# liruiw/OMG-Planner

Measured on AMD Instinct MI355X. Metric: CHOMP iterations/sec (batched scenes) + ms/plan, Panda 7-DoF 30-wp, higher is better.
Workload: dtype f32 SDF / f64 kinematics+update; 1 GPU; 100 table-top scenes/GPU x (64-goal goal-set cost + CHOMP step), Panda 9-dof, 30 waypoints; scenes_per_gpu=100, total_scenes=100, goals=64, waypoints=30, sdf_grid=4x64^3 + 128x96x32 per scene, private, goal_selection=MD on device (omgx_goal_update_optimize), pipeline_parts=3, top_k_collision=1000, plan_restart_every_steps=50

## Files before the change

### include/omg_hip.h

```cpp
#ifndef OMG_HIP_H
#define OMG_HIP_H

#include <stdint.h>

#ifdef __cplusplus
extern "C" {
#endif

#define OMGX_OK 0
#define OMGX_ERR_INVALID (-1)
#define OMGX_ERR_LAUNCH (-2)
#define OMGX_ERR_UNSUPPORTED (-3)

#define OMGX_NUM_LINKS 10
#define OMGX_NUM_DOF 9
#define OMGX_MAX_POINTS 16
#define OMGX_MAX_WAYPOINTS 64
#define OMGX_MAX_CONSTRAINTS 8
#define OMGX_INFO_STRIDE 16

#define OMGX_ROBOT_POSE0 0
#define OMGX_ROBOT_TIP2JOINT 160
#define OMGX_ROBOT_CENTER_OFFSET 320
#define OMGX_ROBOT_JOINT_AXIS 480
// ... 188 lines not shown
                         const int32_t* h_dims, float* out, void* stream);

int32_t omgx_goalset_schedule_len(int32_t num_scenes, int32_t num_goals, int32_t slack);
int omgx_goalset_schedule(const uint32_t* work, const int32_t* active, const int32_t* goal_count, int32_t num_scenes,
                          int32_t num_goals, int32_t slack, int32_t* schedule, void* stream);

int omgx_goalset_schedule_parts(const uint32_t* work, const int32_t* active, const int32_t* goal_count, int32_t num_scenes,
                                int32_t num_goals, int32_t parts, int32_t slack, int32_t* schedule, void* stream);

#define OMGX_SCHEDULE_SCENE_MAJOR 0
#define OMGX_SCHEDULE_LONGEST_FIRST 1
#define OMGX_SCHEDULE_LONGEST_FIRST_MAX_ITEMS 8192
int omgx_goalset_schedule_ordered(const uint32_t* work, const int32_t* active, const int32_t* goal_count, int32_t num_scenes,
                                  int32_t num_goals, int32_t parts, int32_t slack, int32_t order, int32_t* schedule, void* stream);

int64_t omgx_region_scratch_bytes(int32_t dx, int32_t dy, int32_t dz);
int omgx_object_set_grid(omgx_object* object, const float* h_lo, const float* h_hi, const int32_t* h_dims, float delta,
                         int64_t grid_offset, void* stream);
int omgx_fit_influence_region(omgx_object* object, const float* grid, const int32_t* h_dims, const float* h_lo, const float* h_hi,
                              float epsilon, float clearance, void* scratch, void* stream);

int64_t omgx_regions_scratch_bytes(int32_t n_fit, int64_t need_bytes);
int omgx_volume_hashes(const omgx_object* objects, int32_t num_objects, const float* pool, uint64_t* hashes, void* stream);
int omgx_fit_influence_regions(omgx_object* objects, int32_t num_objects, const float* pool, const int32_t* fit_list,
                               const int64_t* need_offsets, int32_t n_fit, int64_t max_voxels, const int32_t* copy_src,
                               void* scratch, void* stream);

typedef struct omgx_plan_iter {
    int32_t mode;
    int32_t start_idx;
// ... 105 lines not shown
```

### omg-planner_amd/csrc/omg_goalset_queue.h

```cpp
#pragma once

#define GQ_TBL_MAX 32
#ifndef GQ_WG_PER_CU
#define GQ_WG_PER_CU 5
#endif
#ifndef GQ_WAVES
#define GQ_WAVES 4
#endif
#define GQ_NT (64 * GQ_WAVES)

struct GqFar {
    float T[12], lo[3], rc[3], rh[3], rr2, rb_r;
    bool cullable;
    int disabled;
};

typedef uint32_t GqU16 __attribute__((ext_vector_type(16)));
typedef uint32_t GqU8 __attribute__((ext_vector_type(8)));
typedef uint32_t GqU4 __attribute__((ext_vector_type(4)));
static_assert(offsetof(omgx_object, pose_inv) == 0 && offsetof(omgx_object, lo) == 0x30 && offsetof(omgx_object, epsilon) == 0x58 &&
              offsetof(omgx_object, clearance) == 0x60 && offsetof(omgx_object, disabled) == 0x64 && offsetof(omgx_object, rb_c) == 0x88 &&
              offsetof(omgx_object, rb_h) == 0x94 && offsetof(omgx_object, rb_r) == 0xa0 && offsetof(omgx_object, rb_r2) == 0xa4 &&
              sizeof(omgx_object) >= 0xa8, "gq_load_far reads the record by byte offsets");
__device__ __forceinline__ GqFar gq_load_far(ObjTablePtr ob) {
// ... 75 lines not shown
    e[12] = __float_as_uint(r.eps); e[13] = __float_as_uint(r.clr);
    e[14] = __float_as_uint(r.pad); e[15] = __float_as_uint(r.i2e);
}

template <bool PERSIST>
__device__ __forceinline__ double gq_ld_traj(const double* p) {
    if constexpr (PERSIST) return __hip_atomic_load(p, __ATOMIC_RELAXED, __HIP_MEMORY_SCOPE_AGENT);
    else return *p;
}
template <bool PERSIST>
__device__ __forceinline__ void gq_st_out(float* p, float v) {
    if constexpr (PERSIST) __hip_atomic_store(p, v, __ATOMIC_RELAXED, __HIP_MEMORY_SCOPE_AGENT);
    else *p = v;
}

template <int LB, bool STAMP, bool LAT, bool SPLIT, bool PRE, bool PERSIST = false, int ROLE = 0, int W = GQ_WAVES, bool RANGE = false>
__device__ __forceinline__ void gq_item(const ChunkArgs& a, double* const lds_pose, const int s, const bool is_layer, const int layer_part, const int chunk, const int NP) {
    const int o_begin = as_const(a.scene_begin)[s], o_end = as_const(a.scene_begin)[s + 1];
    const int P = a.P;
    const bool warming = LAT && o_end > o_begin;
    const int goal = NP > 1 ? chunk / NP : chunk;
    const int part = NP > 1 ? chunk - goal * NP : 0;
    static_assert(!RANGE || (SPLIT && !LAT && !PRE && !PERSIST && W == GQ_WAVES), "waypoint ranges: the batch kernel with two parts per goal and their own kinematics");
    const int CHg = a.CH;
    const int cfg_off = (RANGE && part > 0) ? a.range_h : 0;
    const int CH = RANGE ? (part > 0 ? CHg - a.range_h : a.range_h) : CHg;
    const int blk_shift = (4 - (CH & 3)) & 3;
    const int p = threadIdx.x & 15, lane = threadIdx.x & 63;
    const int wave = __builtin_amdgcn_readfirstlane((int)(threadIdx.x >> 6));
    const int tid = (int)threadIdx.x;
    const RobotViewS rv(a.robot, P);
    const int pstride = a.PS, MR = a.MR;
    static_assert(W == GQ_WAVES || (!LAT && !SPLIT && !PRE && !PERSIST && W >= 4), "wide workgroups: the batch kernel with whole goals and its own kinematics");
    constexpr int NT = 64 * W;
    const GqLayout L(pstride, MR, P, a.tbl_n, LAT, W);
    char* const lds_bytes = reinterpret_cast<char*>(lds_pose);
    uint32_t* const rowmask = reinterpret_cast<uint32_t*>(lds_bytes + L.mask_off);
    uint32_t* const tilebits = reinterpret_cast<uint32_t*>(lds_bytes + L.tile_off);
    if (ROLE == 1 || (ROLE == 0 && is_layer)) {
        const int lgi = a.layer_nb > 1 ? layer_part / a.layer_nb : layer_part, cbi = layer_part - lgi * a.layer_nb;
        const int lpg = 10 / a.layer_lg, c_begin = cbi * a.layer_cb;
        const int c_end = c_begin + a.layer_cb < a.wp_n ? c_begin + a.layer_cb : a.wp_n;
        waypoint_layer_block<LAT, PERSIST>(a, s, lgi * lpg, (lgi + 1) * lpg, c_begin, c_end, lds_pose, rowmask, o_begin, o_end, rv,
                                  reinterpret_cast<double*>(lds_bytes + L.fkc_off), warming,
                                  reinterpret_cast<float*>(lds_bytes + L.objc_off), reinterpret_cast<double*>(lds_bytes + L.btab_off));
        GS_WG_STAMP(4);
        return;
    }
    if (a.goal_count && goal >= as_const(a.goal_count)[s]) {
        if (STAMP && tid == 0) a.work[(int64_t)s * a.NCH + chunk] = 0u;
        return;
    }
    const unsigned long long work_t0 = STAMP ? wall_clock64() : 0ull;
    GS_FREQ_BEGIN();
    uint32_t* const tbl = reinterpret_cast<uint32_t*>(lds_bytes + L.tbl_off);
    double* const pts = reinterpret_cast<double*>(lds_bytes + L.pts_off);
    float* const stage = reinterpret_cast<float*>(lds_bytes + L.stage_off) + wave * 256;

    auto cull_row = [&](int l, int ci) {
        const double* A = lds_pose + 9 + ((int64_t)l * pstride + ci) * 9;
        const auto bl = rv.ball(l);
        float cx, cy, cz;
        link_ball_center(A, A + 3, A + 6, bl, cx, cy, cz);
        const float rad = (float)bl[3] + 1.0e-4f;
// ... 58 lines not shown
            for (int j = 0; j < 12; ++j) {
                const int l = lk / 9, k = lk - 9 * l;
                if (e0 + GQ_NT * j < ne) lds_pose[((size_t)l * pstride + c) * 9 + k] = v[j];
                c += dr; lk += dq;
                if (c >= ncfg) { c -= ncfg; ++lk; }
            }
        }
#pragma unroll
        for (int j = 0; j < 3; ++j) if (tid + GQ_NT * j < nm) rowmask[tid + GQ_NT * j] = mv[j];
        if (tid < 30 * P) pts[tid] = pv0;
        if (tid + GQ_NT < 30 * P) pts[tid + GQ_NT] = pv1;
        if (tbl_lane) gq_tbl_store(tbl + (tid - 128) * 16, trec);
        GS_WG_STAMP(1);
    } else
    {
        const double* q0 = a.traj_start + a.ts_stride * (int64_t)s;
        const double* qg = a.goals + ((int64_t)s * a.NG + goal) * 9;
        const int ncfg = CH + 1;
        double* sc = reinterpret_cast<double*>(lds_bytes + L.stage_off);
        int* const progress = reinterpret_cast<int*>(lds_bytes + L.stage_off + pstride * 14 * 8);
        if (tid < 4) progress[tid] = (tid < chain_waves || (cull_beside_chain && tid == 3)) ? 0 : 99;
        const double pv0 = tid < 30 * P ? rv.g[246 + tid] : 0.0, pv1 = (tid < 256 && tid + 256 < 30 * P) ? rv.g[246 + tid + 256] : 0.0;
        double* const fkc = reinterpret_cast<double*>(lds_bytes + L.fkc_off);
        const double fkv = (LAT && tid < 246) ? rv.g[tid] : 0.0;
        const bool tbl_lane = tid >= 128 && tid - 128 < a.tbl_n && o_begin + tid - 128 < o_end;
        GqTblRec trec{};
        if (LAT && tbl_lane) trec = gq_tbl_load(a.objects + o_begin + (tid - 128));
        if (warming) gq_warm_scalar_cache(a.objects, o_begin, o_end, a.robot + OMGX_ROBOT_POINTS + 30 * P + 316 + 30 * P);
        auto joint = [&](int cfg_local, int d) {
            const int cfg = cfg_local + cfg_off;
            const double q0d = gq_ld_traj<PERSIST>(q0 + d);
            return cfg == 0 ? q0d : q0d + ((double)cfg * (1.0 / (double)(CHg + 1))) * (qg[d] - q0d);
        };
        for (int t = tid; t < ncfg * 7; t += NT) {
            const int cfg = t / 7, i = t - cfg * 7;
            double sn, cs;
#ifdef OMGX_GS_PRO2
            {
                double qq = joint(cfg, i);
                asm volatile("" : "+v"(qq));
                fk_joint_sincos(qq, sn, cs);
                asm volatile("" : : "v"(sn), "v"(cs));
            }
#endif
            fk_joint_sincos(joint(cfg, i), sn, cs);
            sc[2 * t] = sn; sc[2 * t + 1] = cs;
        }
        if (LAT && tid < 246) fkc[tid] = fkv;
        __syncthreads();
        GS_WG_STAMP(1);
        if (tid < 30 * P) pts[tid] = pv0;
        if (tid < 256 && tid + 256 < 30 * P) pts[tid + 256] = pv1;
        if (tbl_lane) {
            if (!LAT) trec = gq_tbl_load(a.objects + o_begin + (tid - 128));
            gq_tbl_store(tbl + (tid - 128) * 16, trec);
        }
        auto run_chain = [&](const auto& view) {
            for (int t = tid; t < ncfg * 3; t += NT) {
                const int cfg = t / 3, rr = t - cfg * 3;
                fk_chain_row(view, rr, sc + 14 * cfg, joint(cfg, 7), joint(cfg, 8), [&](int l, double r0, double r1, double r2, double tr) {
// ... 413 lines not shown
template <int W> struct GqWide { static constexpr int wg_per_cu = W == GQ_WAVES ? GQ_WG_PER_CU : (W <= 6 ? 3 : 2); };
template <int LB, bool STAMP, bool LAT, bool SPLIT, bool PRE, int W, bool RANGE>
__device__ __forceinline__ void goalset_queue_body(const ChunkArgs& a, double* const lds_pose) {
    GS_WG_STAMP(0);
#ifdef OMGX_GS_PRIO
    __builtin_amdgcn_s_setprio(OMGX_GS_PRIO);
#endif
    const int xcd = blockIdx.x & 7;
    const int LPARTS = a.layer_parts;
    const bool spread = LAT;
    static_assert(!(LAT && SPLIT), "latency mode has its parts already");
    const int NP = (LAT || SPLIT) ? a.NP : 1;
    bool is_layer;
    int s, chunk, layer_part;
    bool scheduled = false;
    if (spread) {
        const int nl = a.wp_traj ? a.S * LPARTS : 0;
        is_layer = (int)blockIdx.x < nl;
        const int j = (int)blockIdx.x - nl;
        s = is_layer ? (int)blockIdx.x / LPARTS : j / a.NCH;
        layer_part = (int)blockIdx.x - s * LPARTS;
        chunk = is_layer ? 0 : j - s * a.NCH;
    } else {
        const int nlayer = a.wp_traj ? ((a.S + 7) >> 3) * LPARTS : 0;
        is_layer = (int)(blockIdx.x >> 3) < nlayer;
        const int j = (int)(blockIdx.x >> 3) - nlayer;
        const int sgrp = is_layer ? (int)(blockIdx.x >> 3) / LPARTS : j / a.NCH;
        layer_part = (int)(blockIdx.x >> 3) - sgrp * LPARTS;
        s = sgrp * 8 + xcd;
        chunk = is_layer ? 0 : j - sgrp * a.NCH;
        scheduled = a.schedule && !is_layer;
        if (scheduled) {
            const int item = as_const(a.schedule)[(int)blockIdx.x - nlayer * 8];
            if (item < 0 || item >= a.S * a.NCH) return;
            s = item / a.NCH;
            chunk = item - s * a.NCH;
            if (a.active && as_const(a.active)[s] == 0) { if (STAMP && threadIdx.x == 0) a.work[item] = 0u; return; }
        }
    }
    if (s >= a.S) return;
    if (a.active && !scheduled && !spread) {
        const int k = s, ln = threadIdx.x & 63;
        int seen = 0;
        s = -1;
        for (int base = 0; base < a.S; base += 64) {
            const int i = base + ln;
            const unsigned long long bal = __ballot(i < a.S && a.active[i] != 0);
            const int cnt = __popcll(bal);
            if (k < seen + cnt) {
                unsigned long long m = bal;
                for (int q = k - seen; q > 0; --q) m &= m - 1;
                s = base + __builtin_ctzll(m);
                break;
            }
            seen += cnt;
        }
    }
    if (s < 0) return;
    if (spread && a.active && as_const(a.active)[s] == 0) return;
    if constexpr (W != GQ_WAVES) {
        if (is_layer && threadIdx.x >= 64 * GQ_WAVES) return;
    }
    gq_item<LB, STAMP, LAT, SPLIT, PRE, false, 0, W, RANGE>(a, lds_pose, s, is_layer, layer_part, chunk, NP);
}

template <int LB, bool STAMP = false, bool LAT = false, bool SPLIT = false, bool PRE = false, int W = GQ_WAVES>
__global__ __launch_bounds__(LAT ? 256 : 64 * W, LAT ? 2 : GqWide<W>::wg_per_cu) void k_goalset_queue(ChunkArgs a) {
    extern __shared__ __attribute__((aligned(16))) double lds_pose[];
    goalset_queue_body<LB, STAMP, LAT, SPLIT, PRE, W, false>(a, lds_pose);
}

template <int LB, bool STAMP = false>
__global__ __launch_bounds__(GQ_NT, GQ_WG_PER_CU) void k_goalset_range(ChunkArgs a) {
    extern __shared__ __attribute__((aligned(16))) double lds_pose[];
    goalset_queue_body<LB, STAMP, false, true, false, GQ_WAVES, true>(a, lds_pose);
}
```

### omg-planner_amd/csrc/omg_kernels.hip

```cpp
#include <hip/hip_runtime.h>
#include <hip/hip_ext.h>

#include <stdint.h>
#include <stdio.h>
#include <stdlib.h>
#include <string.h>

#include <mutex>

#include "omg_device.h"
#include "omg_host.h"

using namespace omg;

struct RawObjects {
    const float* __restrict__ pose_init;
    const float* __restrict__ sdf_grids;
    const float* __restrict__ sdf_limits;
    const float* __restrict__ eps;
    const float* __restrict__ pad;
    const float* __restrict__ clr;
    const float* __restrict__ dis;
};

// ... 129 lines not shown
    int wp_n, wp_soften;
    float* wp_pot;
    float* wp_grad;
    float* wp_col;
    int PS, MR;
    const int32_t* schedule;
    int sched_len;
    int tbl_n;
    int NG, NP;
    int range_h;
    int layer_parts, layer_lg, layer_nb, layer_cb, spread;
    double* wp_pose_out;
    uint32_t* work;
    double* pre_poses;
    uint32_t* pre_masks;
};

template <bool WANT_GRAD, int LB, bool FUSED, int TPB = 256>
__global__ __launch_bounds__(TPB) void k_sdf_chunks(ChunkArgs a) {
    extern __shared__ __attribute__((aligned(16))) double lds_pose[];
    __shared__ float red[2][TPB / 64];
    uint32_t* rowmask = reinterpret_cast<uint32_t*>(lds_pose + (FUSED ? (size_t)(a.CH + 1) * 120 : 0));
    const int xcd = blockIdx.x & 7;
    const int nlg = 10 / a.LPW;
    const int jj = blockIdx.x >> 3;
    const int j = jj / nlg, lg = jj - j * nlg;
    const int sgrp = j / a.NCH;
    const int s = sgrp * 8 + xcd, chunk = j - sgrp * a.NCH;
    if (s >= a.S) return;
    const int l_begin = lg * a.LPW, l_end = l_begin + a.LPW;
// ... 643 lines not shown
    }
    ca.pre_poses = nullptr; ca.pre_masks = nullptr;
    if (pre) {
        const int64_t goals = (int64_t)ca.S * ca.NG;
        ca.pre_poses = reinterpret_cast<double*>(tl.kin_ws);
        ca.pre_masks = reinterpret_cast<uint32_t*>(ca.pre_poses + goals * gk_pose_doubles(ca.CH));
        const int ncfg = ca.CH + 1, gpw = ncfg <= 64 ? 64 / ncfg : 1;
        const int64_t waves = (int64_t)ca.S * ((ca.NG + gpw - 1) / gpw);
        hipLaunchKernelGGL(k_goalset_kin, dim3((unsigned)((waves + 3) / 4)), dim3(256), 0, st, ca);
        OMGX_CHECK_LAUNCH("k_goalset_kin");
    }
    hipEvent_t ev0, ev1;
    timing_events(timing_kind, &ev0, &ev1);
    const unsigned g = (unsigned)grid;
    uint32_t l32 = (uint32_t)lds;
#ifdef OMGX_GS_CLOCK
    if (const char* e = getenv("OMGX_GS_LDS_MIN")) { const uint32_t v = (uint32_t)atoi(e); if (v > l32 && v <= 64 * 1024) l32 = v; }
#endif
    const auto go = [&](auto* kernel, int block) { gs_launch(kernel, g, (unsigned)block, l32, st, ev0, ev1, ca); };
    if (range) { if (ca.work) go(k_goalset_range<2, true>, GQ_NT); else go(k_goalset_range<2, false>, GQ_NT); }
    else if (wide == 6) { if (ca.work) go(k_goalset_queue<2, true, false, false, false, 6>, 64 * 6); else go(k_goalset_queue<2, false, false, false, false, 6>, 64 * 6); }
    else if (wide == 8) { if (ca.work) go(k_goalset_queue<2, true, false, false, false, 8>, 64 * 8); else go(k_goalset_queue<2, false, false, false, false, 8>, 64 * 8); }
    else if (ca.spread) { if (pre) go(k_goalset_queue<2, false, true, false, true>, 256); else go(k_goalset_queue<2, false, true, false, false>, 256); }
    else if (split && ca.work) { if (pre) go(k_goalset_queue<2, true, false, true, true>, GQ_NT); else go(k_goalset_queue<2, true, false, true, false>, GQ_NT); }
    else if (split) { if (pre) go(k_goalset_queue<2, false, false, true, true>, GQ_NT); else go(k_goalset_queue<2, false, false, true, false>, GQ_NT); }
    else if (ca.work) { if (pre) go(k_goalset_queue<2, true, false, false, true>, GQ_NT); else go(k_goalset_queue<2, true, false, false, false>, GQ_NT); }
    else { if (pre) go(k_goalset_queue<2, false, false, false, true>, GQ_NT); else go(k_goalset_queue<2, false, false, false, false>, GQ_NT); }
    g_last_goalset_variant = (range ? 0x100 : 0) | (split ? 0x200 : 0) | (ca.spread ? 0x400 : 0) | (pre ? 0x800 : 0) | (range ? GQ_WAVES : wide);
    OMGX_CHECK_LAUNCH("k_goalset_queue");
    return OMGX_OK;
// ... 143 lines not shown

struct GoalsetCall {
    const double* robot = nullptr; int32_t n_points = 0;
    const omgx_object* objects = nullptr; const int32_t* scene_begin = nullptr; const float* sdf_pool = nullptr;
    const double* traj_start = nullptr; int64_t traj_start_stride = 0; const double* goals = nullptr;
    int32_t num_scenes = 0, num_goals = 0, n_remaining = 0, soften_fingers = 0;
    double time_interval = 0.0;
    float *goal_cost = nullptr, *collides = nullptr;
    float* potentials = nullptr;
    void* workspace = nullptr;
    const double* layer_traj = nullptr;
    int32_t layer_n = 0, layer_soften = 0;
    float *layer_pot = nullptr, *layer_grad = nullptr, *layer_col = nullptr;
    const int32_t *active = nullptr, *goal_count = nullptr, *schedule = nullptr;
    int32_t schedule_len = 0; uint32_t* work = nullptr;
    void* stream = nullptr;
    GsTiling tiling;
};

static int goalset_cost_impl(const GoalsetCall& a) {
    if (a.num_scenes < 0 || a.num_goals < 0) return OMGX_ERR_INVALID;
    if (a.num_scenes == 0 || (a.num_goals == 0 && !a.layer_traj)) return OMGX_OK;
    if (!a.robot || !a.objects || !a.scene_begin) return OMGX_ERR_INVALID;
    if (a.num_goals > 0 && (!a.traj_start || !a.goals || !a.goal_cost)) return OMGX_ERR_INVALID;
    if (a.n_points < 1 || a.n_points > OMGX_MAX_POINTS || a.n_remaining < 1 || a.n_remaining > OMGX_MAX_WAYPOINTS)
        return OMGX_ERR_UNSUPPORTED;
    if (!(a.time_interval > 0.0) || (a.num_goals > 0 && a.traj_start_stride < 9)) return OMGX_ERR_INVALID;
    hipStream_t st = (hipStream_t)a.stream;
    const int n = a.num_goals > 0 ? a.n_remaining : 0, C = a.num_goals * n;
    if (a.layer_traj) {
// ... 2 lines not shown
        if (a.potentials) return OMGX_ERR_UNSUPPORTED;
    }
    if ((a.active || a.goal_count || a.schedule || a.work) && a.potentials) return OMGX_ERR_UNSUPPORTED;
    ChunkArgs ca{};
    ca.robot = a.robot; ca.objects = a.objects; ca.scene_begin = a.scene_begin; ca.pool = a.sdf_pool;
    ca.S = a.num_scenes; ca.C = C; ca.CH = n; ca.NCH = a.num_goals; ca.P = a.n_points; ca.soften = a.soften_fingers != 0;
    ca.arc = 1; ca.inv_dt = (float)(1.0 / a.time_interval);
    ca.pot = a.potentials; ca.grad = nullptr; ca.col = nullptr; ca.chunk_cost = a.goal_cost; ca.chunk_col = a.collides;
    ca.traj_start = a.traj_start; ca.ts_stride = a.traj_start_stride; ca.goals = a.goals;
    if (a.layer_traj) {
        ca.wp_traj = a.layer_traj; ca.wp_n = a.layer_n; ca.wp_soften = a.layer_soften != 0;
        ca.wp_pot = a.layer_pot; ca.wp_grad = a.layer_grad; ca.wp_col = a.layer_col;
    }
    if (a.schedule && (a.schedule_len < 8 || a.schedule_len % 8 != 0)) return OMGX_ERR_INVALID;
    ca.active = a.active; ca.goal_count = a.goal_count; ca.schedule = a.schedule; ca.sched_len = a.schedule ? a.schedule_len : 0; ca.work = a.work;
    GsTiling tl = a.tiling;
    tl.kin_ws = a.workspace;
    return a.potentials ? launch_chunks(ca, st) : launch_goalset(ca, 0, st, tl);
}

extern "C" int omgx_goalset_cost(const double* robot, int32_t n_points, const omgx_object* objects,
                                 const int32_t* scene_begin, const float* sdf_pool, const double* traj_start,
                                 int64_t traj_start_stride, const double* goals, int32_t num_scenes, int32_t num_goals,
                                 int32_t n_remaining,
                                 double time_interval, int32_t soften_fingers, float* goal_cost, float* potentials,
                                 float* collides, void* workspace, const int32_t* active, const int32_t* goal_count, void* stream) {
    GoalsetCall a;
    a.robot = robot; a.n_points = n_points; a.objects = objects; a.scene_begin = scene_begin; a.sdf_pool = sdf_pool;
    a.traj_start = traj_start; a.traj_start_stride = traj_start_stride; a.goals = goals; a.num_scenes = num_scenes; a.num_goals = num_goals;
    a.n_remaining = n_remaining; a.time_interval = time_interval; a.soften_fingers = soften_fingers;
// ... 226 lines not shown
                                             float* collides, const double* traj, int32_t n_waypoints,
                                             int32_t layer_soften_fingers, float* layer_potentials, float* layer_grads,
                                             float* layer_collides, const int32_t* active, const int32_t* goal_count,
                                             const int32_t* schedule, int32_t schedule_len, uint32_t* work, int32_t goal_parts,
                                             double* layer_poses, void* workspace, void* stream) {
    if (!traj) return OMGX_ERR_INVALID;
    GoalsetCall a;
    a.robot = robot; a.n_points = n_points; a.objects = objects; a.scene_begin = scene_begin; a.sdf_pool = sdf_pool;
    a.traj_start = traj_start; a.traj_start_stride = traj_start_stride; a.goals = goals; a.num_scenes = num_scenes; a.num_goals = num_goals;
    a.n_remaining = n_remaining; a.time_interval = time_interval; a.soften_fingers = soften_fingers;
    a.goal_cost = goal_cost; a.collides = collides; a.workspace = workspace;
    a.layer_traj = traj; a.layer_n = n_waypoints; a.layer_soften = layer_soften_fingers; a.layer_pot = layer_potentials; a.layer_grad = layer_grads; a.layer_col = layer_collides;
    a.active = active; a.goal_count = goal_count; a.schedule = schedule; a.schedule_len = schedule_len; a.work = work; a.stream = stream;
    a.tiling.goal_parts = goal_parts; a.tiling.wp_pose_out = layer_poses;
    return goalset_cost_impl(a);
}

extern "C" int32_t omgx_goalset_parts(int32_t n_remaining, int32_t goal_parts) {
    if (n_remaining < 1 || goal_parts < 1 || goal_parts > 8) return 0;
    return gs_parts(n_remaining, goal_parts);
}

extern "C" int omgx_goalset_cost_layer_tiled(const double* robot, int32_t n_points, const omgx_object* objects,
                                             const int32_t* scene_begin, const float* sdf_pool, const double* traj_start,
                                             int64_t traj_start_stride, const double* goals, int32_t num_scenes, int32_t num_goals,
                                             int32_t n_remaining, double time_interval, int32_t soften_fingers, float* goal_cost,
                                             float* collides, const double* traj, int32_t n_waypoints, int32_t layer_soften_fingers,
                                             float* layer_potentials, float* layer_grads, float* layer_collides,
                                             const int32_t* active, const int32_t* goal_count, int32_t goal_parts,
                                             int32_t layer_link_groups, int32_t layer_config_block, int32_t spread, double* layer_poses,
// ... 146 lines not shown
```

### omg-planner_amd/engine.py

```python
from __future__ import annotations

import operator
import os

import numpy as np
import torch

from . import _lib, ops
from .config import Config
from .robot import PandaModel
from .scenes import SceneBatch


def shard_range(num_items: int, rank: int, world: int) -> range:
    base, rem = divmod(num_items, world)
    lo = rank * base + min(rank, rem)
    return range(lo, lo + base + (1 if rank < rem else 0))


_SIDE_STREAMS: dict = {}


def _side_stream(device: torch.device, i: int) -> "torch.cuda.Stream":
    key = (device.index if device.index is not None else torch.cuda.current_device(), i)
    st = _SIDE_STREAMS.get(key)
    if st is None:
        st = _SIDE_STREAMS[key] = torch.cuda.Stream(device=device)
    return st


_ALL_DONE_CHECKS = frozenset((1, 2, 3, 5, 8, 13, 21, 34, 55))


class ChompEngine:
    split_update = None
    HOT_FIXED_GOAL = True
    separate_launches = False
    reschedule_every = 0
    schedule_slack = 2
    pipeline = None
    PIPELINE_MIN_ITEMS = 768
    PIPELINE_THREE_BELOW = 16384
    MEASURE_MIN_ITEMS = 256
    LONGEST_FIRST_MAX_ITEMS = 2048

    @classmethod
    def auto_parts(cls, num_scenes: int, num_goals: int) -> int:
        items = num_scenes * num_goals
        if items < cls.PIPELINE_MIN_ITEMS:
            return 1
        return min(num_scenes, 3 if items < cls.PIPELINE_THREE_BELOW else 2)

    SMOOTH_SINGLE_PART_BELOW = int(os.environ.get("OMGX_SMOOTH_SINGLE_PART_BELOW", 32))
    WIDE_WINDOW_FROM = 57
# ... 403 lines not shown

    def _uniform_schedule(self, parts: int = 1) -> torch.Tensor:
        S, G = self.S, self.G * parts
        if self.goal_count is not None:
            items = np.concatenate([s * G + np.arange(int(c) * parts) for s, c in enumerate(self._goal_counts_host)])
        else:
            items = np.arange(S * G)
        n = len(items)
        pos = np.arange(n)
        x = np.minimum(8 * pos // max(n, 1), 7)
        first = np.searchsorted(x, np.arange(8))
        rank = pos - first[x]
        slots = int(rank.max()) + 1 if n else 1
        sched = np.full(slots * 8, -1, np.int32)
        sched[rank * 8 + x] = items
        return torch.as_tensor(sched, device=self.device)

    def build_schedule(self, active: "torch.Tensor | None" = None, uniform: bool = False, parts: int = 1) -> torch.Tensor:
        self._sched_np = parts
        if self.S * self.G * parts > 65536 or self.S > _lib.SCHEDULE_MAX_SCENES:
            if self._uniform_cache is None:
                self._uniform_cache = {}
            if parts not in self._uniform_cache:
                self._uniform_cache[parts] = self._uniform_schedule(parts)
            return self._uniform_cache[parts]
        if self._sched_buf is None:
            self._sched_buf = {}
        self._sched_flip ^= 1
        key = (parts, self._sched_flip)
        out = ops.goalset_schedule(None if uniform else self.work[: self.S * self.G * parts], self.S, self.G, active=active, goal_count=self.goal_count,
                                   slack=self.schedule_slack, out=self._sched_buf.get(key), device=self.device, parts=parts,
                                   longest_first=(not uniform) and self.S * self.G * parts <= self.LONGEST_FIRST_MAX_ITEMS)
        self._sched_buf[key] = out
        return out

    def _layer(self):
        if self.latency:
            ops.goalset_cost_layer_tiled(self.robot, self.P, self.scenes, None, None, 1, self.cfg.time_interval, self.traj,
                                         (self.pot, self.pgrad, self.col), None, layer_soften_fingers=self.cfg.uncheck_finger_collision == -1,
                                         layer_link_groups=self.LAT_LAYER_LINK_GROUPS,
                                         layer_config_block=self.LAT_LAYER_BLOCK, spread=True,
                                         layer_poses=self.wp_pose if self._poses_on else None)
            return
        if self._poses_on:
            ops.goalset_cost_layer_tiled(self.robot, self.P, self.scenes, None, None, 1, self.cfg.time_interval, self.traj,
                                         (self.pot, self.pgrad, self.col), None, layer_soften_fingers=self.cfg.uncheck_finger_collision == -1,
                                         goal_parts=1, layer_link_groups=5, layer_config_block=0, spread=False, layer_poses=self.wp_pose)
# ... 392 lines not shown
```

### omg-planner_amd/ops.py

```python
from __future__ import annotations

import os
import ctypes as C

import numpy as np
import torch

from . import _lib
from ._lib import ChompParams, LearnerParams, check

_ws_cache: dict = {}


def _ptr(t):
    return None if t is None else C.c_void_p(t.data_ptr())


def _stream():
    return C.c_void_p(torch.cuda.current_stream().cuda_stream)


def _need(t: torch.Tensor, dtype, name: str):
    if not t.is_cuda:
        raise _lib.OmgHipError(f"{name} must be a device tensor (the reference asserts CHECK_CUDA, omg_layers.cpp:5)")
# ... 77 lines not shown
def _iteration_tensors(S: int, goal_set, reach, state, goal_idx, cost_vector, start, end, goal_rows, goal_point, step_out, active, goal_count,
                       eta, scene_flags=None):
    for n_, t in (("goal_set", goal_set), ("state", state), ("start", start), ("end", end), ("goal", goal_rows), ("goal_point", goal_point),
                  *zip(("grad", "cost_traj", "info"), step_out)):
        _need(t, torch.float64, n_)
    for n_, t in (("reach", reach), ("cost_vector", cost_vector)):
        if t is not None:
            _need(t, torch.float64, n_)
    if goal_idx.dtype != torch.int32 or not goal_idx.is_cuda or goal_idx.numel() != S:
        raise _lib.OmgHipError("goal_idx must be an int32 device tensor [S]")
    if scene_flags is not None and (scene_flags.dtype != torch.int32 or scene_flags.numel() < S or not scene_flags.is_cuda):
        raise _lib.OmgHipError("scene_flags must be an int32 device tensor [S]")
    _active(active, S); _active(goal_count, S); _eta(eta, S)


def _schedule_args(schedule, work, items: int):
    work = None if work is None else _ptr(_i32n(work, items, "work"))
    if schedule is None:
        return None, 0, work
    return _ptr(_i32n(schedule, None, "schedule")), schedule.numel(), work


class _GoalsetArgs:

    def __init__(self, robot, P, scenes: "DeviceScenes", goals, S, G, dt, soften_fingers, goal_out, layer, layer_soften_fingers, goal_count, kin_ws):
        traj, n, lp, lg, lc, self.poses = layer
        self.scene = (_ptr(robot), int(P), _ptr(scenes.objects), _ptr(scenes.scene_begin), _ptr(scenes.pool))
        self.goals = (_ptr(goals), S, G)
        self.cost = (float(dt), int(bool(soften_fingers)), *goal_out)
        self.layer = (traj, n, int(bool(layer_soften_fingers)), lp, lg, lc)
        self.items, self.goal_count, self.ws = S * G, _ptr(goal_count), _ptr(kin_ws)

    def _args(self, start, n_remaining, ws, active, tail, stream):
        return (*self.scene, *start, *self.goals, n_remaining, *self.cost, *ws, *self.layer, active, self.goal_count, *tail, stream)

    def whole(self, start, n_remaining, active, schedule, work, stream):
        return self._args(start, n_remaining, (self.ws,), active, _schedule_args(schedule, work, self.items), stream)

    def parts(self, start, n_remaining, active, schedule, work, NP, goal_parts, poses, stream):
        return self._args(start, n_remaining, (), active, (*_schedule_args(schedule, work, self.items * NP), goal_parts, poses, self.ws), stream)

    def tiled(self, start, n_remaining, active, tiling, poses, stream):
        return self._args(start, n_remaining, (), active, (*tiling, poses, self.ws), stream)


def sdf_loss_forward(pose_init, sdf_grids, sdf_limits, points, epsilons, padding_scales, clearances, disables):
    for n, t in (("pose_init", pose_init), ("sdf_grids", sdf_grids), ("sdf_limits", sdf_limits), ("points", points),
                 ("epsilons", epsilons), ("padding_scales", padding_scales), ("clearances", clearances), ("disables", disables)):
        _need(t, torch.float32, n)
    N, O = points.shape[0], pose_init.shape[0]
    pot = torch.empty(N, dtype=torch.float32, device=points.device)
    grad = torch.empty((N, 3), dtype=torch.float32, device=points.device)
    col = torch.empty(N, dtype=torch.float32, device=points.device)
    with torch.cuda.device(points.device):
        check(_lib.lib().omgx_sdf_loss_forward(_ptr(pose_init), _ptr(sdf_grids), _ptr(sdf_limits), _ptr(points),
# ... 287 lines not shown
    layer = _layer(S, P, traj, layer_out, layer_poses)
    dev = goals.device
    NP = goalset_parts(n_remaining, goal_parts) if int(goal_parts) != 1 else 1
    if NP < 1:
        raise _lib.OmgHipError("goal_parts must be 1, 2, 4 or 8")
    if out is None:
        cost = torch.empty((S, G) if NP == 1 else (S, G, NP), dtype=torch.float32, device=dev)
        col = torch.empty((S, G) if NP == 1 else (S, G, NP), dtype=torch.float32, device=dev)
    else:
        cost, col = out
    l = _lib.lib()
    with torch.cuda.device(dev):
        g = _GoalsetArgs(robot, P, scenes, goals, S, G, dt, soften_fingers, _goal_out((cost, col), S * G * NP), layer, layer_soften_fingers,
                         _active(goal_count, S), _kin_workspace(prepass, S, G, n_remaining, P, dev))
        active = _ptr(_active(active, S))
        if int(goal_parts) != 1 or layer_poses is not None:
            check(l.omgx_goalset_cost_layer_parts(*g.parts(start, n_remaining, active, schedule, work, NP, int(goal_parts), g.poses, _stream())),
                  "omgx_goalset_cost_layer_parts")
        else:
            check(l.omgx_goalset_cost_layer(*g.whole(start, n_remaining, active, schedule, work, _stream())), "omgx_goalset_cost_layer")
    return cost, col


def goalset_parts(n_remaining: int, goal_parts: int) -> int:
    return int(_lib.lib().omgx_goalset_parts(int(n_remaining), int(goal_parts)))


def goalset_cost_layer_tiled(robot, P, scenes: DeviceScenes, traj_start, goals, n_remaining, dt, traj, layer_out, out,
                             soften_fingers=False, layer_soften_fingers=False, active=None, goal_count=None, goal_parts=4,
                             layer_link_groups=10, layer_config_block=16, spread=True, layer_poses=None, prepass=False):
    dev = (goals if goals is not None else traj).device
# ... 8 lines not shown
            raise _lib.OmgHipError("goal_parts must be 1, 2, 4 or 8")
        goal_out = _goal_out(out, S * G * parts)
    else:
        n_remaining, prepass = 1, None
    layer = _layer(S, P, traj, layer_out, layer_poses)
    with torch.cuda.device(dev):
        g = _GoalsetArgs(robot, P, scenes, goals, S, G, dt, soften_fingers, goal_out, layer, layer_soften_fingers, _active(goal_count, S),
                         _kin_workspace(prepass, S, G, n_remaining, P, dev))
        tiling = (int(goal_parts), int(layer_link_groups), int(layer_config_block), int(bool(spread)))
        check(_lib.lib().omgx_goalset_cost_layer_tiled(*g.tiled(start, int(n_remaining), _ptr(_active(active, S)), tiling, g.poses, _stream())),
              "omgx_goalset_cost_layer_tiled")
    return parts


def goalset_schedule(work, num_scenes: int, num_goals: int, active=None, goal_count=None, slack: int = 2, out=None, device=None,
                     parts: int = 1, longest_first: bool = False):
    l = _lib.lib()
    parts = int(parts)
    n = int(l.omgx_goalset_schedule_len(num_scenes, num_goals * parts, slack))
    if out is None:
        for t in (work, active, goal_count):
            if t is not None:
                device = t.device
                break
        if device is None:
            raise _lib.OmgHipError("goalset_schedule needs a device: pass work, active, goal_count, out or device")
        out = torch.empty(n, dtype=torch.int32, device=device)
    _i32n(out, n, "schedule")
    _i32n(work, num_scenes * num_goals * parts, "work")
    with torch.cuda.device(out.device):
        if longest_first:
            check(l.omgx_goalset_schedule_ordered(_ptr(work), _ptr(_active(active, num_scenes)), _ptr(_active(goal_count, num_scenes)),
                                                  num_scenes, num_goals, parts, slack, _lib.SCHEDULE_LONGEST_FIRST, _ptr(out), _stream()),
                  "omgx_goalset_schedule_ordered")
        elif parts != 1:
            check(l.omgx_goalset_schedule_parts(_ptr(work), _ptr(_active(active, num_scenes)), _ptr(_active(goal_count, num_scenes)),
                                                num_scenes, num_goals, parts, slack, _ptr(out), _stream()), "omgx_goalset_schedule_parts")
        else:
            check(l.omgx_goalset_schedule(_ptr(work), _ptr(_active(active, num_scenes)), _ptr(_active(goal_count, num_scenes)), num_scenes,
                                          num_goals, slack, _ptr(out), _stream()), "omgx_goalset_schedule")
    return out


def forward_kinematics(robot, P, joints, want_joint_info=True):
    _need(joints, torch.float64, "joints")
    B, dev = joints.shape[0], joints.device
    poses = torch.empty((B, 10, 4, 4), dtype=torch.float64, device=dev)
    org = torch.empty((B, 10, 3), dtype=torch.float64, device=dev) if want_joint_info else None
    ax = torch.empty((B, 10, 3), dtype=torch.float64, device=dev) if want_joint_info else None
    with torch.cuda.device(dev):
        check(_lib.lib().omgx_forward_kinematics(_ptr(robot), P, _ptr(joints), B, _ptr(poses), _ptr(org), _ptr(ax), _stream()),
              "omgx_forward_kinematics")
    return poses, org, ax


# ... 166 lines not shown
        n = layer[1]
        self._tiling = None if tiling is None else tuple(int(v) for v in tiling)
        self._goal_parts = int(goal_parts) if self._tiling is None else 1
        max_parts = self._tiling[0] if self._tiling is not None else self._goal_parts
        goal_ptrs = _goal_out(goal_out, S * G * (goalset_parts(n, max_parts) if max_parts != 1 else 1))
        _iteration_tensors(S, goal_set, reach, state, goal_idx, cost_vector, start, end, goal_rows, goal_point, step_out, active, goal_count,
                           eta, scene_flags)
        self.S, self.G, self.n, self.P, self.dt = S, G, n, int(P), float(dt)
        self.device = traj.device
        self._dev_index = traj.device.index if traj.device.index is not None else torch.cuda.current_device()
        self._traj_addr = traj.data_ptr()
        l = _lib.lib()
        self._f_gs, self._f_up = l.omgx_goalset_cost_layer, l.omgx_goal_update_optimize
        self._f_gst = l.omgx_goalset_cost_layer_tiled
        self._f_gsp = l.omgx_goalset_cost_layer_parts
        self.kin_workspace = (torch.empty(max(16, l.omgx_goalset_workspace_bytes(S, G, n, self.P)), dtype=torch.uint8, device=traj.device)
                              if prepass else None)
        self._gs = _GoalsetArgs(robot, P, scenes, goals, S, G, dt, False, goal_ptrs, layer, layer_soften_fingers, goal_count, self.kin_workspace)
        self._layer_alone = _GoalsetArgs(robot, P, scenes, None, S, 0, dt, False, (None, None), layer, layer_soften_fingers, None, None)
        p = _ptr
        self._active_p = p(active)
        traj_p, _n, lp, lg, lc, _poses = layer
        grad, cost_traj, info = step_out
        self._up_a = (p(goal_set), p(reach), goal_ptrs[0], p(state), p(goal_idx), p(cost_vector), p(robot))
        self._up_b = (traj_p, p(start), p(end), p(goal_rows), p(goal_point), lp, lg, lc, p(active), S, p(grad), p(cost_traj), p(info), None)
        self._flags, self._eta = p(scene_flags), p(eta)
        self.use_layer_poses = False

    def goalset_layer(self, start_idx: int, masked: bool, schedule, work, stream):
        g, start, n_remaining = self._gs, (C.c_void_p(self._traj_addr + 72 * start_idx), self.n * 9), self.n - start_idx
        active, poses, stream = self._active_p if masked else None, g.poses if self.use_layer_poses else None, C.c_void_p(stream)
        if self._tiling is not None:
            if schedule is not None or work is not None:
                raise _lib.OmgHipError("a tiled goal-set launch takes no dispatch schedule")
            self._call(self._f_gst, g.tiled(start, n_remaining, active, self._tiling, poses, stream))
        elif self._goal_parts > 1 or self.use_layer_poses:
            NP = goalset_parts(n_remaining, self._goal_parts) if self._goal_parts > 1 else 1
            self._call(self._f_gsp, g.parts(start, n_remaining, active, schedule, work, NP, self._goal_parts, poses, stream))
        else:
            self._call(self._f_gs, g.whole(start, n_remaining, active, schedule, work, stream))

    def _call(self, fn, args):
        if torch.cuda.current_device() == self._dev_index:
            check(fn(*args), fn.__name__)
        else:
            with torch.cuda.device(self.device):
                check(fn(*args), fn.__name__)

    LAYER_ONLY_TILING = tuple(int(x) for x in os.environ["OMGX_LAYER_ONLY_TILING"].split(",")) if os.environ.get("OMGX_LAYER_ONLY_TILING") else None

    def _layer_only_tiling(self):
        if self.LAYER_ONLY_TILING is not None:
# ... 424 lines not shown
```

Before: 557,000 iterations/s.

## Precompute per-workgroup goal item records and hoist entry loads in goal-set kernel

Adds a small kernel that turns the dispatch schedule into 32-byte per-workgroup records holding item, scene, chunk, object range and a padding flag. Goal workgroups can then read everything with one scalar load instead of dependent schedule, scene_begin and goal_count loads. Separately, the start and goal joint values and robot point parameters are loaded at item entry so their latency overlaps earlier setup. The records path is gated behind an engine flag that is off by default, and it adds an extra launch plus Python cache-validation logic.

```diff
diff --git a/include/omg_hip.h b/include/omg_hip.h
--- a/include/omg_hip.h
+++ b/include/omg_hip.h
@@ -226,6 +226,22 @@
 int omgx_goalset_schedule_ordered(const uint32_t* work, const int32_t* active, const int32_t* goal_count, int32_t num_scenes,
                                   int32_t num_goals, int32_t parts, int32_t slack, int32_t order, int32_t* schedule, void* stream);
 
+#define OMGX_GOAL_ITEM_INTS 8
+int omgx_goalset_item_records(const int32_t* schedule, int32_t schedule_len, const int32_t* scene_begin, const int32_t* goal_count,
+                              int32_t num_scenes, int32_t num_goals, int32_t parts, int32_t* records, void* stream);
+int omgx_goalset_cost_layer_items(const double* robot, int32_t n_points,
+                                  const omgx_object* objects, const int32_t* scene_begin, const float* sdf_pool,
+                                  const double* traj_start, int64_t traj_start_stride, const double* goals,
+                                  int32_t num_scenes, int32_t num_goals, int32_t n_remaining,
+                                  double time_interval, int32_t soften_fingers,
+                                  float* goal_cost, float* collides,
+                                  const double* traj, int32_t n_waypoints, int32_t layer_soften_fingers,
+                                  float* layer_potentials, float* layer_grads, float* layer_collides,
+                                  const int32_t* active, const int32_t* goal_count,
+                                  const int32_t* schedule, int32_t schedule_len, uint32_t* work,
+                                  int32_t goal_parts, double* layer_poses, void* workspace,
+                                  const int32_t* records, void* stream);
+
 int64_t omgx_region_scratch_bytes(int32_t dx, int32_t dy, int32_t dz);
 int omgx_object_set_grid(omgx_object* object, const float* h_lo, const float* h_hi, const int32_t* h_dims, float delta,
                          int64_t grid_offset, void* stream);
diff --git a/omg-planner_amd/csrc/omg_goalset_queue.h b/omg-planner_amd/csrc/omg_goalset_queue.h
--- a/omg-planner_amd/csrc/omg_goalset_queue.h
+++ b/omg-planner_amd/csrc/omg_goalset_queue.h
@@ -113,9 +113,16 @@
     else *p = v;
 }
 
+struct GqEntry {
+    bool rec, padded;
+    int o_begin, o_end;
+};
 template <int LB, bool STAMP, bool LAT, bool SPLIT, bool PRE, bool PERSIST = false, int ROLE = 0, int W = GQ_WAVES, bool RANGE = false>
-__device__ __forceinline__ void gq_item(const ChunkArgs& a, double* const lds_pose, const int s, const bool is_layer, const int layer_part, const int chunk, const int NP) {
-    const int o_begin = as_const(a.scene_begin)[s], o_end = as_const(a.scene_begin)[s + 1];
+__device__ __forceinline__ void gq_item(const ChunkArgs& a, double* const lds_pose, const int s, const bool is_layer, const int layer_part, const int chunk, const int NP,
+                                        const GqEntry en = GqEntry{}) {
+    int o_begin, o_end;
+    if (en.rec) { o_begin = en.o_begin; o_end = en.o_end; }
+    else { o_begin = as_const(a.scene_begin)[s]; o_end = as_const(a.scene_begin)[s + 1]; }
     const int P = a.P;
     const bool warming = LAT && o_end > o_begin;
     const int goal = NP > 1 ? chunk / NP : chunk;
@@ -146,7 +153,24 @@
         GS_WG_STAMP(4);
         return;
     }
-    if (a.goal_count && goal >= as_const(a.goal_count)[s]) {
+    constexpr bool ENTRY_LOADS = !PRE && !PERSIST;
+    const double* const q0 = a.traj_start + a.ts_stride * (int64_t)s;
+    const double* const qg = a.goals + ((int64_t)s * a.NG + goal) * 9;
+    const int e_joint = tid - (tid / 7) * 7;
+    double e_q0 = 0.0, e_qg = 0.0, e_pv0 = 0.0, e_pv1 = 0.0;
+    if constexpr (ENTRY_LOADS) {
+        if (tid < (CH + 1) * 7) { e_q0 = q0[e_joint]; e_qg = qg[e_joint]; }
+        if (tid < 30 * P) e_pv0 = rv.g[246 + tid];
+        if (tid < 256 && tid + 256 < 30 * P) e_pv1 = rv.g[246 + tid + 256];
+    }
+    int e_active = 1;
+    if (en.rec && a.active) e_active = as_const(a.active)[s];
+    if (en.rec) {
+        if (e_active == 0 || en.padded) {
+            if (STAMP && tid == 0) a.work[(int64_t)s * a.NCH + chunk] = 0u;
+            return;
+        }
+    } else if (a.goal_count && goal >= as_const(a.goal_count)[s]) {
         if (STAMP && tid == 0) a.work[(int64_t)s * a.NCH + chunk] = 0u;
         return;
     }
@@ -235,27 +259,30 @@
         GS_WG_STAMP(1);
     } else
     {
-        const double* q0 = a.traj_start + a.ts_stride * (int64_t)s;
-        const double* qg = a.goals + ((int64_t)s * a.NG + goal) * 9;
         const int ncfg = CH + 1;
         double* sc = reinterpret_cast<double*>(lds_bytes + L.stage_off);
         int* const progress = reinterpret_cast<int*>(lds_bytes + L.stage_off + pstride * 14 * 8);
         if (tid < 4) progress[tid] = (tid < chain_waves || (cull_beside_chain && tid == 3)) ? 0 : 99;
-        const double pv0 = tid < 30 * P ? rv.g[246 + tid] : 0.0, pv1 = (tid < 256 && tid + 256 < 30 * P) ? rv.g[246 + tid + 256] : 0.0;
+        double pv0 = e_pv0, pv1 = e_pv1;
+        if constexpr (!ENTRY_LOADS) {
+            pv0 = tid < 30 * P ? rv.g[246 + tid] : 0.0;
+            pv1 = (tid < 256 && tid + 256 < 30 * P) ? rv.g[246 + tid + 256] : 0.0;
+        }
         double* const fkc = reinterpret_cast<double*>(lds_bytes + L.fkc_off);
         const double fkv = (LAT && tid < 246) ? rv.g[tid] : 0.0;
         const bool tbl_lane = tid >= 128 && tid - 128 < a.tbl_n && o_begin + tid - 128 < o_end;
         GqTblRec trec{};
         if (LAT && tbl_lane) trec = gq_tbl_load(a.objects + o_begin + (tid - 128));
         if (warming) gq_warm_scalar_cache(a.objects, o_begin, o_end, a.robot + OMGX_ROBOT_POINTS + 30 * P + 316 + 30 * P);
-        auto joint = [&](int cfg_local, int d) {
+        auto joint_of = [&](int cfg_local, double q0d, double qgd) {
             const int cfg = cfg_local + cfg_off;
-            const double q0d = gq_ld_traj<PERSIST>(q0 + d);
-            return cfg == 0 ? q0d : q0d + ((double)cfg * (1.0 / (double)(CHg + 1))) * (qg[d] - q0d);
+            return cfg == 0 ? q0d : q0d + ((double)cfg * (1.0 / (double)(CHg + 1))) * (qgd - q0d);
         };
+        auto joint = [&](int cfg_local, int d) { return joint_of(cfg_local, gq_ld_traj<PERSIST>(q0 + d), qg[d]); };
         for (int t = tid; t < ncfg * 7; t += NT) {
             const int cfg = t / 7, i = t - cfg * 7;
             double sn, cs;
+            const double qi = (ENTRY_LOADS && t == tid) ? joint_of(cfg, e_q0, e_qg) : joint(cfg, i);
 #ifdef OMGX_GS_PRO2
             {
                 double qq = joint(cfg, i);
@@ -264,7 +291,7 @@
                 asm volatile("" : : "v"(sn), "v"(cs));
             }
 #endif
-            fk_joint_sincos(joint(cfg, i), sn, cs);
+            fk_joint_sincos(qi, sn, cs);
             sc[2 * t] = sn; sc[2 * t + 1] = cs;
         }
         if (LAT && tid < 246) fkc[tid] = fkv;
@@ -708,6 +735,7 @@
     bool is_layer;
     int s, chunk, layer_part;
     bool scheduled = false;
+    GqEntry en{};
     if (spread) {
         const int nl = a.wp_traj ? a.S * LPARTS : 0;
         is_layer = (int)blockIdx.x < nl;
@@ -716,23 +744,36 @@
         layer_part = (int)blockIdx.x - s * LPARTS;
         chunk = is_layer ? 0 : j - s * a.NCH;
     } else {
-        const int nlayer = a.wp_traj ? ((a.S + 7) >> 3) * LPARTS : 0;
+        const int nlayer = a.nlayer;
         is_layer = (int)(blockIdx.x >> 3) < nlayer;
-        const int j = (int)(blockIdx.x >> 3) - nlayer;
-        const int sgrp = is_layer ? (int)(blockIdx.x >> 3) / LPARTS : j / a.NCH;
-        layer_part = (int)(blockIdx.x >> 3) - sgrp * LPARTS;
-        s = sgrp * 8 + xcd;
-        chunk = is_layer ? 0 : j - sgrp * a.NCH;
-        scheduled = a.schedule && !is_layer;
-        if (scheduled) {
-            const int item = as_const(a.schedule)[(int)blockIdx.x - nlayer * 8];
-            if (item < 0 || item >= a.S * a.NCH) return;
-            s = item / a.NCH;
-            chunk = item - s * a.NCH;
-            if (a.active && as_const(a.active)[s] == 0) { if (STAMP && threadIdx.x == 0) a.work[item] = 0u; return; }
-        }
-    }
-    if (s >= a.S) return;
+        if (!is_layer && a.records) {
+            typedef const OMG_CONST_AS GqU8* RecPtr;
+            const GqU8 r = *((RecPtr)(uintptr_t)a.records + ((int)blockIdx.x - nlayer * 8));
+            const int item = (int)r[0];
+            if (item < 0 || item >= a.S * a.NCH || (int)r[2] < 0 || (int)r[2] >= a.NCH || (int)r[1] * a.NCH + (int)r[2] != item) return;
+            s = (int)r[1];
+            chunk = (int)r[2];
+            layer_part = 0;
+            scheduled = true;
+            en.rec = true; en.padded = r[5] != 0u;
+            en.o_begin = (int)r[3]; en.o_end = (int)r[4];
+        } else {
+            const int j = (int)(blockIdx.x >> 3) - nlayer;
+            const int sgrp = is_layer ? (int)(blockIdx.x >> 3) / LPARTS : j / a.NCH;
+            layer_part = (int)(blockIdx.x >> 3) - sgrp * LPARTS;
+            s = sgrp * 8 + xcd;
+            chunk = is_layer ? 0 : j - sgrp * a.NCH;
+            scheduled = a.schedule && !is_layer;
+            if (scheduled) {
+                const int item = as_const(a.schedule)[(int)blockIdx.x - nlayer * 8];
+                if (item < 0 || item >= a.S * a.NCH) return;
+                s = item / a.NCH;
+                chunk = item - s * a.NCH;
+                if (a.active && as_const(a.active)[s] == 0) { if (STAMP && threadIdx.x == 0) a.work[item] = 0u; return; }
+            }
+        }
+    }
+    if (!en.rec && s >= a.S) return;
     if (a.active && !scheduled && !spread) {
         const int k = s, ln = threadIdx.x & 63;
         int seen = 0;
@@ -755,7 +796,7 @@
     if constexpr (W != GQ_WAVES) {
         if (is_layer && threadIdx.x >= 64 * GQ_WAVES) return;
     }
-    gq_item<LB, STAMP, LAT, SPLIT, PRE, false, 0, W, RANGE>(a, lds_pose, s, is_layer, layer_part, chunk, NP);
+    gq_item<LB, STAMP, LAT, SPLIT, PRE, false, 0, W, RANGE>(a, lds_pose, s, is_layer, layer_part, chunk, NP, en);
 }
 
 template <int LB, bool STAMP = false, bool LAT = false, bool SPLIT = false, bool PRE = false, int W = GQ_WAVES>
diff --git a/omg-planner_amd/csrc/omg_kernels.hip b/omg-planner_amd/csrc/omg_kernels.hip
--- a/omg-planner_amd/csrc/omg_kernels.hip
+++ b/omg-planner_amd/csrc/omg_kernels.hip
@@ -167,6 +167,8 @@
     uint32_t* work;
     double* pre_poses;
     uint32_t* pre_masks;
+    const int32_t* records;
+    int nlayer;
 };
 
 template <bool WANT_GRAD, int LB, bool FUSED, int TPB = 256>
@@ -840,6 +842,10 @@
     timing_events(timing_kind, &ev0, &ev1);
     const unsigned g = (unsigned)grid;
     uint32_t l32 = (uint32_t)lds;
+    ca.nlayer = (layer && !ca.spread) ? scene_groups * ca.layer_parts : 0;
+    static const int records_on = [] { const char* e = getenv("OMGX_GS_RECORDS"); return e ? atoi(e) : 1; }();
+    if (!ca.schedule || ca.spread || !records_on) ca.records = nullptr;
+    if (ca.records && ((uintptr_t)ca.records & 31)) return OMGX_ERR_INVALID;
 #ifdef OMGX_GS_CLOCK
     if (const char* e = getenv("OMGX_GS_LDS_MIN")) { const uint32_t v = (uint32_t)atoi(e); if (v > l32 && v <= 64 * 1024) l32 = v; }
 #endif
@@ -1013,6 +1019,7 @@
     float *layer_pot = nullptr, *layer_grad = nullptr, *layer_col = nullptr;
     const int32_t *active = nullptr, *goal_count = nullptr, *schedule = nullptr;
     int32_t schedule_len = 0; uint32_t* work = nullptr;
+    const int32_t* records = nullptr;
     void* stream = nullptr;
     GsTiling tiling;
 };
@@ -1045,6 +1052,8 @@
     }
     if (a.schedule && (a.schedule_len < 8 || a.schedule_len % 8 != 0)) return OMGX_ERR_INVALID;
     ca.active = a.active; ca.goal_count = a.goal_count; ca.schedule = a.schedule; ca.sched_len = a.schedule ? a.schedule_len : 0; ca.work = a.work;
+    if (a.records && !a.schedule) return OMGX_ERR_INVALID;
+    ca.records = a.records;
     GsTiling tl = a.tiling;
     tl.kin_ws = a.workspace;
     return a.potentials ? launch_chunks(ca, st) : launch_goalset(ca, 0, st, tl);
@@ -1301,6 +1310,56 @@
     a.active = active; a.goal_count = goal_count; a.schedule = schedule; a.schedule_len = schedule_len; a.work = work; a.stream = stream;
     a.tiling.goal_parts = goal_parts; a.tiling.wp_pose_out = layer_poses;
     return goalset_cost_impl(a);
+}
+
+extern "C" int omgx_goalset_cost_layer_items(const double* robot, int32_t n_points, const omgx_object* objects,
+                                             const int32_t* scene_begin, const float* sdf_pool, const double* traj_start,
+                                             int64_t traj_start_stride, const double* goals, int32_t num_scenes, int32_t num_goals,
+                                             int32_t n_remaining, double time_interval, int32_t soften_fingers, float* goal_cost,
+                                             float* collides, const double* traj, int32_t n_waypoints,
+                                             int32_t layer_soften_fingers, float* layer_potentials, float* layer_grads,
+                                             float* layer_collides, const int32_t* active, const int32_t* goal_count,
+                                             const int32_t* schedule, int32_t schedule_len, uint32_t* work, int32_t goal_parts,
+                                             double* layer_poses, void* workspace, const int32_t* records, void* stream) {
+    if (!traj) return OMGX_ERR_INVALID;
+    GoalsetCall a;
+    a.robot = robot; a.n_points = n_points; a.objects = objects; a.scene_begin = scene_begin; a.sdf_pool = sdf_pool;
+    a.traj_start = traj_start; a.traj_start_stride = traj_start_stride; a.goals = goals; a.num_scenes = num_scenes; a.num_goals = num_goals;
+    a.n_remaining = n_remaining; a.time_interval = time_interval; a.soften_fingers = soften_fingers;
+    a.goal_cost = goal_cost; a.collides = collides; a.workspace = workspace;
+    a.layer_traj = traj; a.layer_n = n_waypoints; a.layer_soften = layer_soften_fingers; a.layer_pot = layer_potentials; a.layer_grad = layer_grads; a.layer_col = layer_collides;
+    a.active = active; a.goal_count = goal_count; a.schedule = schedule; a.schedule_len = schedule_len; a.work = work; a.stream = stream;
+    a.tiling.goal_parts = goal_parts; a.tiling.wp_pose_out = layer_poses;
+    a.records = records;
+    return goalset_cost_impl(a);
+}
+
+static_assert(OMGX_GOAL_ITEM_INTS == 8, "a goal workgroup reads its record by one 32-byte scalar load");
+__global__ __launch_bounds__(256) void k_goalset_item_records(const int32_t* schedule, int n, const int32_t* scene_begin, const int32_t* goal_count,
+                                                              int S, int NCH, int parts, int4* records) {
+    const int k = (int)(blockIdx.x * 256 + threadIdx.x);
+    if (k >= n) return;
+    const int item = schedule[k];
+    int4 lo = make_int4(-1, 0, 0, 0), hi = make_int4(0, 1, 0, 0);
+    if (item >= 0 && item < S * NCH) {
+        const int s = item / NCH, chunk = item - s * NCH;
+        lo = make_int4(item, s, chunk, scene_begin[s]);
+        hi = make_int4(scene_begin[s + 1], (goal_count && chunk / parts >= goal_count[s]) ? 1 : 0, 0, 0);
+    }
+    records[2 * (int64_t)k] = lo;
+    records[2 * (int64_t)k + 1] = hi;
+}
+
+extern "C" int omgx_goalset_item_records(const int32_t* schedule, int32_t schedule_len, const int32_t* scene_begin, const int32_t* goal_count,
+                                         int32_t num_scenes, int32_t num_goals, int32_t parts, int32_t* records, void* stream) {
+    if (!schedule || !scene_begin || !records || schedule_len < 8 || schedule_len % 8 != 0 || num_scenes <= 0 || num_goals <= 0) return OMGX_ERR_INVALID;
+    if (parts != 1 && parts != 2 && parts != 4 && parts != 8) return OMGX_ERR_INVALID;
+    if ((uintptr_t)records & 31) return OMGX_ERR_INVALID;
+    if ((int64_t)num_scenes * num_goals * parts > 0x7fffffff) return OMGX_ERR_UNSUPPORTED;
+    hipLaunchKernelGGL(k_goalset_item_records, dim3((unsigned)((schedule_len + 255) / 256)), dim3(256), 0, (hipStream_t)stream, schedule, (int)schedule_len,
+                       scene_begin, goal_count, (int)num_scenes, (int)(num_goals * parts), (int)parts, reinterpret_cast<int4*>(records));
+    OMGX_CHECK_LAUNCH("k_goalset_item_records");
+    return OMGX_OK;
 }
 
 extern "C" int32_t omgx_goalset_parts(int32_t n_remaining, int32_t goal_parts) {
diff --git a/omg-planner_amd/engine.py b/omg-planner_amd/engine.py
--- a/omg-planner_amd/engine.py
+++ b/omg-planner_amd/engine.py
@@ -38,6 +38,7 @@
     separate_launches = False
     reschedule_every = 0
     schedule_slack = 2
+    item_records = False
     pipeline = None
     PIPELINE_MIN_ITEMS = 768
     PIPELINE_THREE_BELOW = 16384
@@ -471,7 +472,10 @@
         slots = int(rank.max()) + 1 if n else 1
         sched = np.full(slots * 8, -1, np.int32)
         sched[rank * 8 + x] = items
-        return torch.as_tensor(sched, device=self.device)
+        out = torch.as_tensor(sched, device=self.device)
+        if self.item_records:
+            ops.goalset_item_records(out, self.scenes, S, self.G, goal_count=self.goal_count, parts=parts)
+        return out
 
     def build_schedule(self, active: "torch.Tensor | None" = None, uniform: bool = False, parts: int = 1) -> torch.Tensor:
         self._sched_np = parts
@@ -487,7 +491,8 @@
         key = (parts, self._sched_flip)
         out = ops.goalset_schedule(None if uniform else self.work[: self.S * self.G * parts], self.S, self.G, active=active, goal_count=self.goal_count,
                                    slack=self.schedule_slack, out=self._sched_buf.get(key), device=self.device, parts=parts,
-                                   longest_first=(not uniform) and self.S * self.G * parts <= self.LONGEST_FIRST_MAX_ITEMS)
+                                   longest_first=(not uniform) and self.S * self.G * parts <= self.LONGEST_FIRST_MAX_ITEMS,
+                                   scenes=self.scenes if self.item_records else None)
         self._sched_buf[key] = out
         return out
 
diff --git a/omg-planner_amd/ops.py b/omg-planner_amd/ops.py
--- a/omg-planner_amd/ops.py
+++ b/omg-planner_amd/ops.py
@@ -115,6 +115,24 @@
     _active(active, S); _active(goal_count, S); _eta(eta, S)
 
 
+def _records_key(schedule, scene_begin, goal_count, S: int, items_per_scene: int):
+    return (schedule.data_ptr(), schedule._version, scene_begin.data_ptr(), scene_begin._version,
+            None if goal_count is None else (goal_count.data_ptr(), goal_count._version), int(S), int(items_per_scene))
+
+
+def goalset_item_records(schedule, scenes: "DeviceScenes", num_scenes: int, num_goals: int, goal_count=None, parts: int = 1, out=None):
+    _i32n(schedule, None, "schedule")
+    n = schedule.numel()
+    if out is None or out.numel() != n * 8:
+        out = torch.empty((n, 8), dtype=torch.int32, device=schedule.device)
+    _i32n(out, n * 8, "records")
+    with torch.cuda.device(schedule.device):
+        check(_lib.lib().omgx_goalset_item_records(_ptr(schedule), n, _ptr(scenes.scene_begin), _ptr(_active(goal_count, num_scenes)), int(num_scenes),
+                                                   int(num_goals), int(parts), _ptr(out), _stream()), "omgx_goalset_item_records")
+    schedule.item_records = (out, _records_key(schedule, scenes.scene_begin, goal_count, num_scenes, num_goals * int(parts)))
+    return out
+
+
 def _schedule_args(schedule, work, items: int):
     work = None if work is None else _ptr(_i32n(work, items, "work"))
     if schedule is None:
@@ -131,6 +149,8 @@
         self.cost = (float(dt), int(bool(soften_fingers)), *goal_out)
         self.layer = (traj, n, int(bool(layer_soften_fingers)), lp, lg, lc)
         self.items, self.goal_count, self.ws = S * G, _ptr(goal_count), _ptr(kin_ws)
+        self._S, self._G, self._scene_begin, self._goal_count = S, G, scenes.scene_begin, goal_count
+        self._rec_seen = None
 
     def _args(self, start, n_remaining, ws, active, tail, stream):
         return (*self.scene, *start, *self.goals, n_remaining, *self.cost, *ws, *self.layer, active, self.goal_count, *tail, stream)
@@ -140,6 +160,22 @@
 
     def parts(self, start, n_remaining, active, schedule, work, NP, goal_parts, poses, stream):
         return self._args(start, n_remaining, (), active, (*_schedule_args(schedule, work, self.items * NP), goal_parts, poses, self.ws), stream)
+
+    def records(self, schedule, NP):
+        rec = getattr(schedule, "item_records", None) if schedule is not None else None
+        if rec is None:
+            return None
+        gc, c = self._goal_count, self._rec_seen
+        now = (schedule._version, self._scene_begin._version, None if gc is None else gc._version, NP, rec[0])
+        if c is not None and c[0] is schedule and c[1] == now[:4] and c[2] is rec[0]:
+            return rec[0]
+        if rec[1] != _records_key(schedule, self._scene_begin, gc, self._S, self._G * NP):
+            return None
+        self._rec_seen = (schedule, now[:4], rec[0])
+        return rec[0]
+
+    def with_items(self, start, n_remaining, active, schedule, work, NP, goal_parts, poses, records, stream):
+        return self._args(start, n_remaining, (), active, (*_schedule_args(schedule, work, self.items * NP), goal_parts, poses, self.ws, _ptr(records)), stream)
 
     def tiled(self, start, n_remaining, active, tiling, poses, stream):
         return self._args(start, n_remaining, (), active, (*tiling, poses, self.ws), stream)
@@ -457,7 +493,11 @@
         g = _GoalsetArgs(robot, P, scenes, goals, S, G, dt, soften_fingers, _goal_out((cost, col), S * G * NP), layer, layer_soften_fingers,
                          _active(goal_count, S), _kin_workspace(prepass, S, G, n_remaining, P, dev))
         active = _ptr(_active(active, S))
-        if int(goal_parts) != 1 or layer_poses is not None:
+        records = g.records(schedule, NP)
+        if records is not None:
+            check(l.omgx_goalset_cost_layer_items(*g.with_items(start, n_remaining, active, schedule, work, NP, int(goal_parts), g.poses, records, _stream())),
+                  "omgx_goalset_cost_layer_items")
+        elif int(goal_parts) != 1 or layer_poses is not None:
             check(l.omgx_goalset_cost_layer_parts(*g.parts(start, n_remaining, active, schedule, work, NP, int(goal_parts), g.poses, _stream())),
                   "omgx_goalset_cost_layer_parts")
         else:
@@ -496,7 +536,7 @@
 
 
 def goalset_schedule(work, num_scenes: int, num_goals: int, active=None, goal_count=None, slack: int = 2, out=None, device=None,
-                     parts: int = 1, longest_first: bool = False):
+                     parts: int = 1, longest_first: bool = False, scenes: "DeviceScenes | None" = None):
     l = _lib.lib()
     parts = int(parts)
     n = int(l.omgx_goalset_schedule_len(num_scenes, num_goals * parts, slack))
@@ -521,6 +561,9 @@
         else:
             check(l.omgx_goalset_schedule(_ptr(work), _ptr(_active(active, num_scenes)), _ptr(_active(goal_count, num_scenes)), num_scenes,
                                           num_goals, slack, _ptr(out), _stream()), "omgx_goalset_schedule")
+    old = out.__dict__.pop("item_records", None)
+    if scenes is not None:
+        goalset_item_records(out, scenes, num_scenes, num_goals, goal_count=goal_count, parts=parts, out=None if old is None else old[0])
     return out
 
 
@@ -717,6 +760,7 @@
         self._f_gs, self._f_up = l.omgx_goalset_cost_layer, l.omgx_goal_update_optimize
         self._f_gst = l.omgx_goalset_cost_layer_tiled
         self._f_gsp = l.omgx_goalset_cost_layer_parts
+        self._f_gsi = l.omgx_goalset_cost_layer_items
         self.kin_workspace = (torch.empty(max(16, l.omgx_goalset_workspace_bytes(S, G, n, self.P)), dtype=torch.uint8, device=traj.device)
                               if prepass else None)
         self._gs = _GoalsetArgs(robot, P, scenes, goals, S, G, dt, False, goal_ptrs, layer, layer_soften_fingers, goal_count, self.kin_workspace)
@@ -737,8 +781,12 @@
             if schedule is not None or work is not None:
                 raise _lib.OmgHipError("a tiled goal-set launch takes no dispatch schedule")
             self._call(self._f_gst, g.tiled(start, n_remaining, active, self._tiling, poses, stream))
+            return
+        NP = goalset_parts(n_remaining, self._goal_parts) if self._goal_parts > 1 else 1
+        records = g.records(schedule, NP)
+        if records is not None:
+            self._call(self._f_gsi, g.with_items(start, n_remaining, active, schedule, work, NP, self._goal_parts, poses, records, stream))
         elif self._goal_parts > 1 or self.use_layer_poses:
-            NP = goalset_parts(n_remaining, self._goal_parts) if self._goal_parts > 1 else 1
             self._call(self._f_gsp, g.parts(start, n_remaining, active, schedule, work, NP, self._goal_parts, poses, stream))
         else:
             self._call(self._f_gs, g.whole(start, n_remaining, active, schedule, work, stream))
```

After: 548,900 iterations/s. 0.986x the previous value.
